# dyollb/segmantic

Hardware: AMD Instinct MI355X
Metric: 3D UNet train voxels/s on 128^3 bf16 (higher is better)
Workload: dtype bf16

## Files before the change

include/segmi.h:

```cpp
#ifndef SEGMI_H_
#define SEGMI_H_

#include <stddef.h>
#include <stdint.h>

#ifdef __cplusplus
extern "C" {
#endif

#define SEGMI_VERSION 1

enum { SEGMI_F32 = 0, SEGMI_BF16 = 1, SEGMI_F16 = 2 };
enum { SEGMI_OK = 0, SEGMI_EINVAL = -1, SEGMI_EUNSUPPORTED = -2, SEGMI_ELAUNCH = -3,
       SEGMI_EDATA = -4  };

typedef struct segmi_act {
  void* data;
  int32_t n, d, h, w;
  int32_t c;
  int32_t ld;
} segmi_act;

int segmi_version(void);
const char* segmi_last_error(void);
// ... 64 lines not shown
                     const segmi_bn_bwd_sums* bn_bwd ,
                     const segmi_bn_fin* stats_fin , void* stream);
int segmi_dectop_ok(int dtype, const segmi_act* in, const segmi_act* out);
int segmi_dectop_fwd(int dtype, const segmi_act* in, const segmi_act* out, const void* up_frag,
                     const float* up_bias, const float* up_alpha,
                     int up_alpha_in_unit_range ,
                     const void* conv_packed, const float* conv_bias, void* stream);
typedef struct segmi_windows {
  int32_t count;
  int32_t row_stride;
  int64_t plane_stride;
  int64_t offset[32];
} segmi_windows;
int segmi_conv3d_pair_ok(int dtype, const segmi_act* in, const segmi_act* out_a,
                         const segmi_act* out_b);
int segmi_conv3d_split_act_ok(int dtype, const segmi_act* in, const segmi_act* out, int ksize,
                              int stride);
int segmi_conv3d_fwd_split_act(int dtype, const segmi_act* in, const segmi_act* out,
                               const void* packed, const float* bias, const float* prelu_alpha,
                               int act_channels, int ksize, int stride,
                               const float* bias_b , float* stats_partials ,
                               const segmi_bn_fin* stats_fin , void* stream);
int segmi_conv3d_fwd_pair(int dtype, const segmi_act* in, const segmi_act* out_a, const float* w_a,
                          const float* bias_a, const float* prelu_alpha_a, float* stats_partials_a,
                          const segmi_act* out_b, const float* w_b, const float* bias_b, int stride,
                          const segmi_bn_fin* stats_fin_a ,
                          const segmi_windows* windows ,
                          void* stream);

int segmi_convT3d_stats_rows(int dtype, const segmi_act* in, const segmi_act* out);
int segmi_convT3d_fwd(int dtype, const segmi_act* in, const segmi_act* out, const void* packed,
                      const float* w_src, const float* bias, const float* prelu_alpha,
                      const segmi_act* residual, float* stats_partials,
                      const segmi_bn_fin* stats_fin , void* stream);

int64_t segmi_conv3d_wgrad_workspace(int dtype, const segmi_act* x, const segmi_act* dy,
                                     int ksize, int stride, int cus);
int segmi_conv3d_wgrad(int dtype, const segmi_act* x, const segmi_act* dy, float* dw,
                       float* db, int ksize, int stride, void* workspace,
                       const segmi_in_affine* in_tf , int cus, void* stream);
int segmi_wgrad_cus(int cus);
int segmi_bias_grad(int dtype, const segmi_act* dy, float* db, void* workspace, void* stream);

int segmi_bn_stats_rows(const segmi_act* x);
int segmi_bn_stats(int dtype, const segmi_act* x, float* stats_partials, void* stream);
int segmi_bn_finalize(const float* stats_partials, int rows, int c, double count,
                      const float* gamma, const float* beta, float* running_mean,
                      float* running_var, float momentum, float eps, float* mean,
                      float* invstd, float* scale, float* shift, void* stream);
int segmi_bn_eval_affine(int c, const float* gamma, const float* beta,
                         const float* running_mean, const float* running_var, float eps,
                         float* scale, float* shift, void* stream);
int segmi_bn_act_fwd(int dtype, const segmi_act* x, const segmi_act* y, const float* scale,
                     const float* shift, const float* prelu_alpha, const segmi_act* residual,
                     float dropout_p, uint32_t dropout_seed, void* stream);
int segmi_bn_act_bwd_rows(const segmi_act* x);
int segmi_bn_act_bwd_reduce(int dtype, const segmi_act* dy, const segmi_act* x,
                            const float* mean, const float* invstd, const float* gamma,
                            const float* beta, const float* prelu_alpha, float* red_partials,
                            float dropout_p, uint32_t dropout_seed,
                            const segmi_bn_bwd_fin* fin , void* stream);
int segmi_bn_act_bwd_finalize(const float* red_partials, int rows, int c, double count,
                              const float* gamma, const float* invstd, float* dgamma,
                              float* dbeta, float* dalpha, float* coef, void* stream);
int segmi_bn_act_bwd_fused_ok(int dtype, const segmi_act* dy, const segmi_act* x, const segmi_act* dx);
int segmi_bn_act_bwd_fused_rows(const segmi_act* x);
int segmi_bn_act_bwd_fused_wgs(int dtype, const segmi_act* x, int max_wgs);
int segmi_bn_act_bwd_fused(int dtype, const segmi_act* dy, const segmi_act* x, const segmi_act* dx,
                           const float* mean, const float* invstd, const float* gamma, const float* beta,
                           const float* prelu_alpha, float* red_partials, const segmi_bn_bwd_fin* fin,
                           int max_wgs, void* stream);
unsigned segmi_fused_timeouts(int reset);
int segmi_fused_test_hook(unsigned poll_limit, int no_publish);
int segmi_bn_act_bwd_apply(int dtype, const segmi_act* dy, const segmi_act* x,
                           const segmi_act* dx, const float* mean, const float* invstd,
                           const float* gamma, const float* beta, const float* prelu_alpha,
                           const float* coef, float dropout_p, uint32_t dropout_seed, void* stream);
int segmi_bn_act_bwd_apply_conv_ok(int dtype, const segmi_act* dy, const segmi_act* x, const segmi_act* dx,
                                   const segmi_act* out);
int segmi_bn_act_bwd_apply_conv(int dtype, const segmi_act* dy, const segmi_act* x, const segmi_act* dx,
                                const float* mean, const float* invstd, const float* gamma, const float* beta,
                                const float* prelu_alpha, const float* coef, const segmi_act* out,
                                const void* packed, void* stream);

int segmi_add(int dtype, const segmi_act* a, const segmi_act* b, const segmi_act* out,
              void* stream);
int segmi_cast_copy(int src_dtype, const segmi_act* src, int dst_dtype, const segmi_act* dst,
                    void* stream);
int segmi_nchw_to_ndhwc(const float* src, int dst_dtype, const segmi_act* dst, void* stream);
int segmi_ndhwc_to_nchw(int src_dtype, const segmi_act* src, float* dst, void* stream);

int segmi_dice_chunks(const segmi_act* logits);
int segmi_softmax_dice_fwd(int dtype, const segmi_act* logits, const float* labels,
                           float* partials, float* coef, float* loss, float smooth_nr,
                           float smooth_dr, void* stream);
int segmi_softmax_dice_bwd(int dtype, const segmi_act* logits, const float* labels,
                           const float* coef, float grad_scale, const segmi_act* dlogits,
                           float* scratch, float* bias_grad, void* stream);

int segmi_adam_step(float* param, const float* grad, float* exp_avg, float* exp_avg_sq,
                    float* max_exp_avg_sq, int64_t n, double lr, double beta1, double beta2,
                    double eps, double weight_decay, int64_t step, float grad_scale,
                    void* stream);
int segmi_sgd_step(float* param, const float* grad, float* momentum_buf, int64_t n, double lr,
                   double momentum, double weight_decay, int first_step, float grad_scale,
                   void* stream);
int segmi_adabelief_step(float* param, const float* grad, float* exp_avg, float* exp_avg_var,
                         int64_t n, double lr, double beta1, double beta2, double eps,
                         double weight_decay, int weight_decouple, int64_t step,
                         float grad_scale, void* stream);

int segmi_softmax_dice_bwd_amp(int dtype, const segmi_act* logits, const float* labels,
                               const float* coef, const float* amp, const segmi_act* dlogits,
                               float* scratch, float* bias_grad, void* stream);
int segmi_amp_check_finite(const float* grad, int64_t n, float* amp, void* stream);
int segmi_amp_update_scale(float* amp, int32_t* growth_tracker, int64_t* step, double growth_factor,
                           double backoff_factor, int growth_interval, void* stream);
int segmi_adam_step_amp(float* param, const float* grad, float* exp_avg, float* exp_avg_sq,
                        float* max_exp_avg_sq, int64_t n, double lr, double beta1, double beta2,
                        double eps, double weight_decay, const float* amp, const int64_t* step,
                        float grad_scale, void* stream);
int segmi_sgd_step_amp(float* param, const float* grad, float* momentum_buf, int64_t n, double lr,
                       double momentum, double weight_decay, const float* amp, const int64_t* step,
                       float grad_scale, void* stream);
int segmi_adabelief_step_amp(float* param, const float* grad, float* exp_avg, float* exp_avg_var,
                             int64_t n, double lr, double beta1, double beta2, double eps,
                             double weight_decay, int weight_decouple, const float* amp,
                             const int64_t* step, float grad_scale, void* stream);

int segmi_sw_gather(int dtype_src, const segmi_act* image, int img_index,
                    const int32_t* starts_host, int nwin, int dst_dtype,
                    const segmi_act* windows, void* stream);
int segmi_sw_scatter_add(int dtype, const segmi_act* pred, const int32_t* starts_host,
                         int nwin, const float* importance, const segmi_act* acc, float* cnt,
                         void* stream);
int segmi_sw_finalize(const segmi_act* acc, const float* cnt, int write_logits, void* labels,
                      int label_bytes, void* stream);
int segmi_sw_blend(int dtype, const void* cache, int k, int ldp, const int32_t* starts_z, int nz,
                   const int32_t* starts_y, int ny, const int32_t* starts_x, int nx, int win_lo,
                   int win_hi, int rd, int rh, int rw, const float* importance, int d, int h, int w,
                   float* out_logits, int ldo, float* out_count, void* labels, int label_bytes,
                   int normalize, void* stream);
int segmi_argmax(int dtype, const segmi_act* logits, void* labels, int label_bytes,
                 void* stream);
int segmi_label_counts(const int32_t* pred, const int32_t* truth, int64_t n, int k,
                       int64_t* counts, void* stream);

int segmi_resample3d(int pixel, const void* src, int sx, int sy, int sz, void* dst, int dx,
                     int dy, int dz, const double* index_map_host, int interp,
                     double default_value, void* stream);
int64_t segmi_normalize_workspace(int c, int64_t nvox);
int segmi_normalize_intensity(float* x, int c, int64_t nvox, void* workspace, void* stream);
int segmi_crop_patches(const segmi_act* image, const float* label, const int32_t* starts_host,
                       const uint8_t* flips_host, int count, int dst_dtype,
                       const segmi_act* out_image, float* out_label, void* stream);
int segmi_warp_crop_patches(const segmi_act* image, const float* label, const int32_t* starts_host,
                            const uint8_t* flips_host, int count, const double* index_map_host,
                            int dst_dtype, const segmi_act* out_image, float* out_label,
                            void* stream);
int64_t segmi_intensity_workspace(int count);
int segmi_intensity_augment(float* patches, int count, int rd, int rh, int rw, int c,
                            const uint8_t* contrast_on_host, const float* gamma_host,
                            const uint8_t* hist_on_host, const float* ctrl_host, int nctrl,
                            const uint8_t* bias_on_host, const float* coef_host, void* workspace,
                            void* stream);
int64_t segmi_kspace_workspace(int count, int rd, int rh, int rw);
// ... 70 lines not shown
```

segmantic_amd/_lib.py:

```python
from __future__ import annotations

import ctypes as C
import os
from pathlib import Path

import torch

SEGMI_F32 = 0
SEGMI_BF16 = 1
SEGMI_F16 = 2

_LIB_PATH = Path(__file__).resolve().parent / "csrc" / "libsegmi.so"


class Act(C.Structure):

    _fields_ = [("data", C.c_void_p), ("n", C.c_int32), ("d", C.c_int32), ("h", C.c_int32),
                ("w", C.c_int32), ("c", C.c_int32), ("ld", C.c_int32)]


class WpackDesc(C.Structure):

    _fields_ = [("w_src", C.c_void_p), ("scale", C.c_void_p), ("packed", C.c_void_p),
                ("kind", C.c_int32), ("cin_k", C.c_int32), ("cout_k", C.c_int32),
# ... 4 lines not shown
class InAffine(C.Structure):

    _fields_ = [("scale", C.c_void_p), ("shift", C.c_void_p), ("prelu_alpha", C.c_void_p)]


class Windows(C.Structure):

    _fields_ = [("count", C.c_int32), ("row_stride", C.c_int32), ("plane_stride", C.c_int64),
                ("offset", C.c_int64 * 32)]


class BnFin(C.Structure):

    _fields_ = [("count", C.c_double), ("gamma", C.c_void_p), ("beta", C.c_void_p),
                ("running_mean", C.c_void_p), ("running_var", C.c_void_p), ("momentum", C.c_float),
                ("eps", C.c_float), ("mean", C.c_void_p), ("invstd", C.c_void_p), ("scale", C.c_void_p),
                ("shift", C.c_void_p)]


class BnBwdFin(C.Structure):

    _fields_ = [("count", C.c_double), ("dgamma", C.c_void_p), ("dbeta", C.c_void_p), ("dalpha", C.c_void_p),
                ("coef", C.c_void_p)]


class BnBwdSums(C.Structure):

    _fields_ = [("x", C.POINTER(Act)), ("mean", C.c_void_p), ("invstd", C.c_void_p), ("gamma", C.c_void_p),
                ("beta", C.c_void_p), ("prelu_alpha", C.c_void_p), ("partials", C.c_void_p),
                ("fin", C.POINTER(BnBwdFin))]


_P = C.c_void_p
_AP = C.POINTER(Act)
_i = C.c_int
_i64 = C.c_int64
_f = C.c_float
_d = C.c_double

SIGNATURES = {
    "segmi_version": (_i, []),
    "segmi_last_error": (C.c_char_p, []),
    "segmi_stream_create_cumask": (_i, [_i, C.POINTER(C.c_void_p)]),
    "segmi_stream_destroy": (_i, [_P]),
    "segmi_wpack_bytes": (_i64, [_i, _i, _i, _i, _i]),
    "segmi_wpack": (_i, [_i, _i, _P, _P, _i, _i, _i, _P, _P]),
    "segmi_wpack_batch": (_i, [_i, C.POINTER(WpackDesc), _i, _P, _i, _P]),
    "segmi_conv3d_stats_rows": (_i, [_i, _AP, _AP, _i, _i]),
    "segmi_conv3d_in_affine_ok": (_i, [_i, _AP, _AP, _i, _i]),
    "segmi_conv3d_fwd_kernel_name": (C.c_char_p, [_i, _AP, _AP, _i, _i]),
    "segmi_conv3d_split_act_ok": (_i, [_i, _AP, _AP, _i, _i]),
    "segmi_conv3d_fwd_split_act": (_i, [_i, _AP, _AP, _P, _P, _P, _i, _i, _i, _P, _P, C.POINTER(BnFin), _P]),
    "segmi_conv3d_fwd": (_i, [_i, _AP, _AP, _P, _P, _i, _P, _P, _AP, _P, _i, _i, C.POINTER(InAffine),
                              C.POINTER(BnBwdSums), C.POINTER(BnFin), _P]),
    "segmi_conv3d_bn_bwd_sums_ok": (_i, [_i, _AP, _AP, _i, _i]),
    "segmi_dectop_ok": (_i, [_i, _AP, _AP]),
    "segmi_dectop_fwd": (_i, [_i, _AP, _AP, _P, _P, _P, _i, _P, _P, _P]),
    "segmi_conv3d_pair_ok": (_i, [_i, _AP, _AP, _AP]),
    "segmi_conv3d_fwd_pair": (_i, [_i, _AP, _AP, _P, _P, _P, _P, _AP, _P, _P, _i, C.POINTER(BnFin),
                                   C.POINTER(Windows), _P]),
    "segmi_convT3d_stats_rows": (_i, [_i, _AP, _AP]),
    "segmi_convT3d_fwd": (_i, [_i, _AP, _AP, _P, _P, _P, _P, _AP, _P, C.POINTER(BnFin), _P]),
    "segmi_conv3d_wgrad_workspace": (_i64, [_i, _AP, _AP, _i, _i, _i]),
    "segmi_conv3d_wgrad": (_i, [_i, _AP, _AP, _P, _P, _i, _i, _P, C.POINTER(InAffine), _i, _P]),
    "segmi_bias_grad": (_i, [_i, _AP, _P, _P, _P]),
    "segmi_bn_stats_rows": (_i, [_AP]),
    "segmi_bn_stats": (_i, [_i, _AP, _P, _P]),
    "segmi_bn_finalize": (_i, [_P, _i, _i, _d, _P, _P, _P, _P, _f, _f, _P, _P, _P, _P, _P]),
    "segmi_bn_eval_affine": (_i, [_i, _P, _P, _P, _P, _f, _P, _P, _P]),
    "segmi_bn_act_fwd": (_i, [_i, _AP, _AP, _P, _P, _P, _AP, _f, C.c_uint32, _P]),
    "segmi_bn_act_bwd_rows": (_i, [_AP]),
    "segmi_bn_act_bwd_reduce": (_i, [_i, _AP, _AP, _P, _P, _P, _P, _P, _P, _f, C.c_uint32,
                                     C.POINTER(BnBwdFin), _P]),
    "segmi_bn_act_bwd_finalize": (_i, [_P, _i, _i, _d, _P, _P, _P, _P, _P, _P, _P]),
    "segmi_bn_act_bwd_fused_ok": (_i, [_i, _AP, _AP, _AP]),
    "segmi_bn_act_bwd_fused_rows": (_i, [_AP]),
    "segmi_bn_act_bwd_fused": (_i, [_i, _AP, _AP, _AP, _P, _P, _P, _P, _P, _P, C.POINTER(BnBwdFin), _i, _P]),
    "segmi_bn_act_bwd_fused_wgs": (_i, [_i, _AP, _i]),
    "segmi_fused_timeouts": (C.c_uint, [_i]),
    "segmi_fused_test_hook": (_i, [C.c_uint, _i]),
    "segmi_bn_act_bwd_apply": (_i, [_i, _AP, _AP, _AP, _P, _P, _P, _P, _P, _P, _f, C.c_uint32, _P]),
    "segmi_bn_act_bwd_apply_conv_ok": (_i, [_i, _AP, _AP, _AP, _AP]),
    "segmi_bn_act_bwd_apply_conv": (_i, [_i, _AP, _AP, _AP, _P, _P, _P, _P, _P, _P, _AP, _P, _P]),
    "segmi_wgrad_cus": (_i, [_i]),
    "segmi_add": (_i, [_i, _AP, _AP, _AP, _P]),
    "segmi_cast_copy": (_i, [_i, _AP, _i, _AP, _P]),
    "segmi_nchw_to_ndhwc": (_i, [_P, _i, _AP, _P]),
    "segmi_ndhwc_to_nchw": (_i, [_i, _AP, _P, _P]),
    "segmi_dice_chunks": (_i, [_AP]),
    "segmi_softmax_dice_fwd": (_i, [_i, _AP, _P, _P, _P, _P, _f, _f, _P]),
    "segmi_softmax_dice_bwd": (_i, [_i, _AP, _P, _P, _f, _AP, _P, _P, _P]),
    "segmi_adam_step": (_i, [_P, _P, _P, _P, _P, _i64, _d, _d, _d, _d, _d, _i64, _f, _P]),
    "segmi_sgd_step": (_i, [_P, _P, _P, _i64, _d, _d, _d, _i, _f, _P]),
    "segmi_adabelief_step": (_i, [_P, _P, _P, _P, _i64, _d, _d, _d, _d, _d, _i, _i64, _f, _P]),
    "segmi_softmax_dice_bwd_amp": (_i, [_i, _AP, _P, _P, _P, _AP, _P, _P, _P]),
    "segmi_amp_check_finite": (_i, [_P, _i64, _P, _P]),
    "segmi_amp_update_scale": (_i, [_P, _P, _P, _d, _d, _i, _P]),
    "segmi_adam_step_amp": (_i, [_P, _P, _P, _P, _P, _i64, _d, _d, _d, _d, _d, _P, _P, _f, _P]),
    "segmi_sgd_step_amp": (_i, [_P, _P, _P, _i64, _d, _d, _d, _P, _P, _f, _P]),
    "segmi_adabelief_step_amp": (_i, [_P, _P, _P, _P, _i64, _d, _d, _d, _d, _d, _i, _P, _P, _f, _P]),
    "segmi_sw_gather": (_i, [_i, _AP, _i, _P, _i, _i, _AP, _P]),
    "segmi_sw_scatter_add": (_i, [_i, _AP, _P, _i, _P, _AP, _P, _P]),
    "segmi_sw_finalize": (_i, [_AP, _P, _i, _P, _i, _P]),
    "segmi_sw_blend": (_i, [_i, _P, _i, _i, _P, _i, _P, _i, _P, _i, _i, _i, _i, _i, _i, _P, _i, _i, _i,
                            _P, _i, _P, _P, _i, _i, _P]),
    "segmi_argmax": (_i, [_i, _AP, _P, _i, _P]),
    "segmi_label_counts": (_i, [_P, _P, _i64, _i, _P, _P]),
    "segmi_resample3d": (_i, [_i, _P, _i, _i, _i, _P, _i, _i, _i, _P, _i, _d, _P]),
    "segmi_normalize_workspace": (_i64, [_i, _i64]),
    "segmi_normalize_intensity": (_i, [_P, _i, _i64, _P, _P]),
    "segmi_crop_patches": (_i, [_AP, _P, _P, _P, _i, _i, _AP, _P, _P]),
    "segmi_warp_crop_patches": (_i, [_AP, _P, _P, _P, _i, _P, _i, _AP, _P, _P]),
    "segmi_intensity_workspace": (_i64, [_i]),
    "segmi_intensity_augment": (_i, [_P, _i, _i, _i, _i, _i, _P, _P, _P, _P, _i, _P, _P, _P, _P]),
    "segmi_ensemble_mean": (_i, [_P, _P, _i, _i64, _P, _P]),
    "segmi_ensemble_vote": (_i, [_P, _i, _i64, _P, _P]),
    "segmi_ensemble_select": (_i, [_P, _i, _P, _P, _i, _i64, _P, _P]),
    "segmi_kspace_workspace": (_i64, [_i, _i, _i, _i]),
    "segmi_kspace_augment": (_i, [_P, _i, _i, _i, _i, _i, _P, _P, _P, _P, _P, _P, _P, _P]),
    "segmi_label_boxes": (_i, [_P, _P, _i, _i, _i, _i, _i, _P, _P, _P]),
    "segmi_edt_workspace_bytes": (_i64, [_i, _i, _i]),
    "segmi_edt_sq": (_i, [_P, _i, _i, _i, _i, _i, _i, _i, _P, _P, _P, _P, C.c_size_t, _P]),
    "segmi_edt_sample": (_i, [_P, _P, _i, _i, _i, _i, _i, _i, _i, _P, _P, _P, _P, _P, C.c_size_t, _P]),
    "segmi_select_workspace_bytes": (_i64, [_i]),
    "segmi_select_f32": (_i, [_P, _P, _P, _i, _P, _P, C.c_size_t, _P]),
    "segmi_confusion_counts": (_i, [_P, _P, _i, _i64, _i, _P, _P]),
    "segmi_nyul_workspace_bytes": (_i64, [_i, _i]),
    "segmi_nyul_landmarks": (_i, [_P, _i, _i64, _i, _P, _i, _P, _P, _P, C.c_size_t, _P]),
    "segmi_nyul_apply": (_i, [_P, _i, _i64, _i, _P, _P, _P, _i, _P]),
    "segmi_label_centroids": (_i, [_P, _i, _i, _i, _i, _i, _P, _P, _P]),
    "segmi_vert_heatmap": (_i, [_P, _i, _P, _P, _i, _i, _i, _i, _P, _P]),
    "segmi_channel_argmax": (_i, [_P, _i, _i, _i, _i, _P, _P, _P]),
    "segmi_positive_bbox": (_i, [_P, _i, _i, _i, _i, _i, _i, _P, _P]),
    "segmi_otsu_workspace_bytes": (_i64, [_i]),
    "segmi_otsu": (_i, [_P, _i64, _i, _P, _P, _P, C.c_size_t, _P]),
    "segmi_n4_shrink": (_i, [_P, _i, _i, _i, _i, _i, _i, _P, _P, _i, _i, _P, _P, _P, _P]),
    "segmi_n4_workspace_bytes": (_i64, [_i, _i, _i, _i, _i, _i]),
    "segmi_n4_fit": (_i, [_P, _i, _i, _i, _P, _i, _i, _i, _d, _d, _d, _P, _P, _P, _P, _P, C.c_size_t, _P]),
    "segmi_n4_sharpen": (_i, [_P, _i, _i, _i, _i, _d, _d, _P, _P, _P, C.c_size_t, _P]),
    "segmi_n4_bspline_fit": (_i, [_P, _i, _i, _i, _i, _P, _P, C.c_size_t, _P]),
    "segmi_n4_refine": (_i, [_P, _i, _i, _i, _P, _P]),
    "segmi_n4_evaluate": (_i, [_P, _i, _i, _i, _P, _P, _i, _i, _i, _P]),
    "segmi_ct_scale": (_i, [_P, _i, _i, _i, _P, _P]),
}


def _load():
    path = Path(os.environ.get("SEGMI_LIB", str(_LIB_PATH)))
    if not path.exists():
        raise ImportError(
            f"segmantic_amd: native library {path} not found. Build it with "
            f"`python -c 'import __graft_entry__ as g; g.build()'` or `make -C segmantic_amd/csrc`. "
            f"There is no CPU fallback.")
    try:
        lib = C.CDLL(str(path))
    except OSError as e:
        raise ImportError(f"segmantic_amd: cannot load {path}: {e}") from e
    missing = []
    for name, (res, args) in SIGNATURES.items():
        try:
            fn = getattr(lib, name)
        except AttributeError:
            missing.append(name)
            continue
        fn.restype = res
        fn.argtypes = args
# ... 16 lines not shown
```

segmantic_amd/csrc/conv.hip:

```cpp
#include "conv_fwd_impl.h"
#include "conv_ring_impl.h"
#include "conv_ks_impl.h"
#include "convt_ps_impl.h"
#include "conv_bnbwd_impl.h"

namespace segmi {

int conv_s2_bnbwd_bf16(const ConvBnBwdParams& p, hipStream_t st);
int conv_s2_bnbwd_f16(const ConvBnBwdParams& p, hipStream_t st);

int conv_mfma_f32(const ConvParams& p, int ksize, int stride, hipStream_t st);
int conv_mfma_bf16(const ConvParams& p, int ksize, int stride, hipStream_t st);
int conv_mfma_f16(const ConvParams& p, int ksize, int stride, hipStream_t st);
int convt_mfma_f32(const ConvTParams& p, hipStream_t st);
int convt_mfma_bf16(const ConvTParams& p, hipStream_t st);
int convt_mfma_f16(const ConvTParams& p, hipStream_t st);
static inline int conv_mfma_dt(int dtype, const ConvParams& p, int ksize, int stride, hipStream_t st) {
  if (dtype == SEGMI_F32) return conv_mfma_f32(p, ksize, stride, st);
  return dtype == SEGMI_F16 ? conv_mfma_f16(p, ksize, stride, st) : conv_mfma_bf16(p, ksize, stride, st);
}
static inline int convt_mfma_dt(int dtype, const ConvTParams& p, hipStream_t st) {
  if (dtype == SEGMI_F32) return convt_mfma_f32(p, st);
  return dtype == SEGMI_F16 ? convt_mfma_f16(p, st) : convt_mfma_bf16(p, st);
}
int bn_stats_launch(int dtype, const segmi_act* x, float* partials, hipStream_t st, const BiasFin* bias_fin = nullptr);
int bn_stats_rows_for(const segmi_act* x);
int stats_reserve_rows();
static inline int bn_finalize_with(const float* partials, int rows, int c, const segmi_bn_fin* f, hipStream_t st) {
  return segmi_bn_finalize(partials, rows, c, f->count, f->gamma, f->beta, f->running_mean, f->running_var,
                           f->momentum, f->eps, f->mean, f->invstd, f->scale, f->shift, st);
}
bool conv_small_ok(int cin, int cout, int ksize);
int conv_small_fwd(int dtype, const segmi_act* in, const segmi_act* out, const float* w,
                   const float* bias, const float* alpha, const segmi_act* res, float* stats,
                   int stride, hipStream_t st, const segmi_act* out2 = nullptr,
                   const float* w2 = nullptr, const float* bias2 = nullptr,
                   const segmi_bn_fin* fin = nullptr, const segmi_windows* win = nullptr);
int conv_small_fwd_rows(const segmi_act* out);

struct DirectParams {
  const void* in;
  void* out;
  const float* w;
  const float* bias;
  const float* alpha;
  const void* res;
  int N, Di, Hi, Wi, Do, Ho, Wo, Cin, Cout, ldi, ldo, ldr;
  int ks, stride, kind;
};

template <typename T>
__global__ void conv_direct_kernel(DirectParams p) {
  const int64_t total = (int64_t)p.N * p.Do * p.Ho * p.Wo * p.Cout;
  const int pad = (p.ks - 1) / 2, nt = p.ks * p.ks * p.ks;
  const T* in = (const T*)p.in;
  for (int64_t e = blockIdx.x * (int64_t)blockDim.x + threadIdx.x; e < total;
       e += (int64_t)gridDim.x * blockDim.x) {
    const int co = e % p.Cout;
    int64_t v = e / p.Cout;
    const int ox = v % p.Wo; v /= p.Wo;
    const int oy = v % p.Ho; v /= p.Ho;
    const int oz = v % p.Do;
    const int n = v / p.Do;
    float acc = 0.f;
    for (int kd = 0; kd < p.ks; ++kd) {
      const int z = oz * p.stride - pad + kd;
      if ((unsigned)z >= (unsigned)p.Di) continue;
      for (int kh = 0; kh < p.ks; ++kh) {
        const int y = oy * p.stride - pad + kh;
        if ((unsigned)y >= (unsigned)p.Hi) continue;
        for (int kw = 0; kw < p.ks; ++kw) {
          const int x = ox * p.stride - pad + kw;
          if ((unsigned)x >= (unsigned)p.Wi) continue;
          const int tap = (kd * p.ks + kh) * p.ks + kw;
          const T* ip = in + ((((int64_t)n * p.Di + z) * p.Hi + y) * p.Wi + x) * p.ldi;
          if (p.kind == 0) {
            const float* wp = p.w + ((int64_t)co * p.Cin) * nt + tap;
            for (int ci = 0; ci < p.Cin; ++ci) acc = fmaf(Elem<T>::ld(ip + ci), wp[(int64_t)ci * nt], acc);
          } else {
            const float* wp = p.w + (int64_t)co * nt + (nt - 1 - tap);
            for (int ci = 0; ci < p.Cin; ++ci)
              acc = fmaf(Elem<T>::ld(ip + ci), wp[(int64_t)ci * p.Cout * nt], acc);
          }
        }
      }
    }
    if (p.bias) acc += p.bias[co];
// ... 128 lines not shown
                  "conv3d_fwd_split_act: act_channels must be a multiple of 16 within the output channels");
  SEGMI_CHECK_ARG(in->n == out->n && out->d == out_extent(in->d, ksize, stride) &&
                      out->h == out_extent(in->h, ksize, stride) && out->w == out_extent(in->w, ksize, stride),
                  "conv3d_fwd_split_act: output extent does not match the input");
  const int es = dtype_size(dtype);
  SEGMI_CHECK_ARG(in->ld % (16 / es) == 0 && out->ld % 4 == 0 && ((uintptr_t)in->data % 16) == 0 &&
                      ((uintptr_t)out->data % (4 * es)) == 0,
                  "conv3d_fwd_split_act: MFMA path needs 16-byte aligned input rows");
  ConvParams p{};
  p.in = in->data; p.out = out->data; p.wfrag = packed; p.bias = bias; p.alpha = prelu_alpha;
  p.N = in->n; p.Di = in->d; p.Hi = in->h; p.Wi = in->w;
  p.Do = out->d; p.Ho = out->h; p.Wo = out->w;
  p.Cin = in->c; p.Cout = out->c; p.ldi = in->ld; p.ldo = out->ld;
  p.nchunks = in->c / pick_ck(dtype, in->c);
  p.ntiles_total = out->c / 16;
  p.act_tiles = act_channels / 16;
  p.bias2 = bias_b;
  if (stats_partials) {
    p.stats = stats_partials;
    p.stats_tiles = act_channels / 16;
    if (stats_fin) { p.fin_on = 1; p.bfin = bn_fin_from(stats_fin, act_channels); }
  } else {
    SEGMI_CHECK_ARG(!stats_fin, "conv3d_fwd_split_act: stats_fin needs stats_partials");
  }
  hipStream_t st = (hipStream_t)stream;
  return conv_mfma_dt(dtype, p, ksize, stride, st);
}

const char* segmi_conv3d_fwd_kernel_name(int dtype, const segmi_act* in, const segmi_act* out,
                                         int ksize, int stride) {
  static thread_local char buf[96];
  if (!act_ok(in) || !act_ok(out)) return "invalid";
  const char* dt = dtype == SEGMI_BF16 ? "bf16" : dtype == SEGMI_F16 ? "f16" : "f32";
  if (mfma_ok(in->c, out->c)) {
    const int ck = pick_ck(dtype, in->c);
    if (conv_ring_ok(dtype, in->c, ksize, stride, out)) {
      if (conv_ring3_shape_ok(in->c, out->c, in->data, out->data, in->d, in->h, in->w, in->ld, out->d, out->h, out->w, out->ld,
                              out->ld, out->ld))
        snprintf(buf, sizeof buf, "conv_ring3_kernel<%s, CK=16> (LDS-DMA ring)", dt);
      else
        snprintf(buf, sizeof buf, "conv_ring2_kernel<%s, CK=%d, NT=%d>", dt, ck,
                 ck == 32 && (out->c / 16) % 2 == 0 ? 2 : 1);
    }
    else if (conv_ks_ok(dtype, in->c, ksize, stride))
      snprintf(buf, sizeof buf, "conv_fwd_ks_kernel<%s, k%d s%d>", dt, ksize, stride);
    else
      snprintf(buf, sizeof buf, "conv_fwd_mfma_kernel<%s, CK=%d, k%d s%d>", dt, ck, ksize, stride);
    return buf;
  }
  if (small_fwd_eligible(dtype, in, out, ksize)) snprintf(buf, sizeof buf, "conv_small_fwd_kernel<%s>", dt);
  else snprintf(buf, sizeof buf, "conv_direct_kernel<%s>", dt);
  return buf;
}

int segmi_conv3d_in_affine_ok(int dtype, const segmi_act* in, const segmi_act* out, int ksize,
                              int stride) {
  if (!act_ok(in) || !act_ok(out) || !dtype_h16(dtype) || !mfma_ok(in->c, out->c)) return 0;
  return ksize == 3 && stride == 1 && conv_ring_ok(dtype, in->c, ksize, stride, out) ? 1 : 0;
}

int segmi_conv3d_bn_bwd_sums_ok(int dtype, const segmi_act* in, const segmi_act* out, int ksize,
                                int stride) {
  if (!act_ok(in) || !act_ok(out) || !dtype_h16(dtype)) return 0;
  return ((in->c == 16 && out->c == 16) || (in->c == 32 && out->c == 32)) && ksize == 3 && stride == 1 &&
                 conv_ring_ok(dtype, in->c, ksize, stride, out) ? 1 : 0;
}

int segmi_bn_act_bwd_apply_conv_ok(int dtype, const segmi_act* dy, const segmi_act* x, const segmi_act* dx,
                                   const segmi_act* out) {
  if (!dtype_h16(dtype) || !act_ok(dy) || !act_ok(x) || !act_ok(dx) || !act_ok(out)) return 0;
  const segmi_act* a3[3] = {dy, x, dx};
  for (const segmi_act* a : a3) {
    if (a->n != dy->n || a->d != dy->d || a->h != dy->h || a->w != dy->w || a->c != 16) return 0;
    if (a->ld % 8 != 0 || ((uintptr_t)a->data % 16) != 0) return 0;
  }
  if (out->n != dy->n || out->d != out_extent(dy->d, 3, 2) || out->h != out_extent(dy->h, 3, 2) ||
      out->w != out_extent(dy->w, 3, 2))
    return 0;
  if (!(out->c == 16 || out->c == 32 || out->c == 64) || out->ld % 4 != 0 || ((uintptr_t)out->data % 8) != 0)
    return 0;
  const int64_t vox = (int64_t)dy->d * dy->h * dy->w;
  if (vox * dy->ld * 2 >= (1ll << 31) || vox * x->ld * 2 >= (1ll << 31) || vox * dx->ld * 2 >= (1ll << 31)) return 0;
  return out->w >= 16 ? 1 : 0;
}

int segmi_bn_act_bwd_apply_conv(int dtype, const segmi_act* dy, const segmi_act* x, const segmi_act* dx,
                                const float* mean, const float* invstd, const float* gamma, const float* beta,
                                const float* prelu_alpha, const float* coef, const segmi_act* out,
                                const void* packed, void* stream) {
  SEGMI_CHECK_ARG(segmi_bn_act_bwd_apply_conv_ok(dtype, dy, x, dx, out) && mean && invstd && coef && packed,
                  "bn_act_bwd_apply_conv: not eligible (ask segmi_bn_act_bwd_apply_conv_ok) or bad arguments");
  SEGMI_CHECK_ARG(dx->data != dy->data && dx->data != x->data,
                  "bn_act_bwd_apply_conv: dx must not alias dy or x (halo voxels are re-read by neighbouring tiles)");
  ConvBnBwdParams p{};
  p.dy = dy->data; p.x = x->data; p.dx = dx->data; p.out = out->data; p.wfrag = packed;
  p.mean = mean; p.invstd = invstd; p.gamma = gamma; p.beta = beta; p.alpha = prelu_alpha; p.coef = coef;
  p.N = dy->n; p.Di = dy->d; p.Hi = dy->h; p.Wi = dy->w; p.Do = out->d; p.Ho = out->h; p.Wo = out->w;
  p.Cout = out->c; p.ldy = dy->ld; p.ldx = x->ld; p.lddx = dx->ld; p.ldo = out->ld;
  p.ntiles_total = out->c / 16;
  return dtype == SEGMI_F16 ? conv_s2_bnbwd_f16(p, (hipStream_t)stream) : conv_s2_bnbwd_bf16(p, (hipStream_t)stream);
}

int segmi_conv3d_fwd(int dtype, const segmi_act* in, const segmi_act* out, const void* packed,
                     const float* w_src, int w_kind, const float* bias,
                     const float* prelu_alpha, const segmi_act* residual,
                     float* stats_partials, int ksize, int stride, const segmi_in_affine* in_tf,
                     const segmi_bn_bwd_sums* bn_bwd, const segmi_bn_fin* stats_fin, void* stream) {
  SEGMI_CHECK_ARG(!stats_fin || (stats_partials && bn_fin_ok(stats_fin)),
                  "conv3d: stats_fin needs stats_partials and its output pointers");
  if (bn_bwd && bn_bwd->fin)
    SEGMI_CHECK_ARG(bn_bwd->fin->count > 0 && bn_bwd->fin->coef, "conv3d: bn_bwd->fin needs count and coef");
  if (bn_bwd)
    SEGMI_CHECK_ARG(bn_bwd->x && act_ok(bn_bwd->x) && bn_bwd->mean && bn_bwd->invstd && bn_bwd->partials &&
                        segmi_conv3d_bn_bwd_sums_ok(dtype, in, out, ksize, stride) && !prelu_alpha &&
                        !stats_partials && bn_bwd->x->n == out->n && bn_bwd->x->d == out->d &&
                        bn_bwd->x->h == out->h && bn_bwd->x->w == out->w && bn_bwd->x->c == out->c &&
                        bn_bwd->x->ld % 4 == 0 && ((uintptr_t)bn_bwd->x->data % 8) == 0,
                    "conv3d: this launch cannot take BatchNorm-backward sums (ask segmi_conv3d_bn_bwd_sums_ok)");
  if (in_tf)
    SEGMI_CHECK_ARG(in_tf->scale && in_tf->shift && segmi_conv3d_in_affine_ok(dtype, in, out, ksize, stride),
                    "conv3d: this layer cannot take an input transform (ask segmi_conv3d_in_affine_ok)");
  SEGMI_CHECK_ARG(dtype_ok(dtype), "conv3d: bad dtype %d", dtype);
  SEGMI_CHECK_ARG(act_ok(in) && act_ok(out), "conv3d: bad activation view");
  SEGMI_CHECK_ARG((ksize == 1 || ksize == 3) && (stride == 1 || stride == 2),
                  "conv3d: unsupported ksize/stride %d/%d", ksize, stride);
  SEGMI_CHECK_ARG(!(ksize == 1 && stride != 1), "conv3d: k1 is stride 1 only");
  SEGMI_CHECK_ARG(in->n == out->n && out->d == out_extent(in->d, ksize, stride) &&
                      out->h == out_extent(in->h, ksize, stride) &&
                      out->w == out_extent(in->w, ksize, stride),
                  "conv3d: output extent [%d,%d,%d,%d] does not match input [%d,%d,%d,%d] k%d s%d",
                  out->n, out->d, out->h, out->w, in->n, in->d, in->h, in->w, ksize, stride);
  if (residual)
    SEGMI_CHECK_ARG(act_ok(residual) && residual->n == out->n && residual->d == out->d &&
                        residual->h == out->h && residual->w == out->w && residual->c == out->c,
                    "conv3d: residual shape mismatch");
  hipStream_t st = (hipStream_t)stream;
  const int es = dtype_size(dtype);
  if (mfma_ok(in->c, out->c)) {
    SEGMI_CHECK_ARG(packed, "conv3d: MFMA path needs a fragment-packed weight (segmi_wpack)");
    SEGMI_CHECK_ARG(in->ld % (16 / es) == 0 && out->ld % 4 == 0 &&
                        ((uintptr_t)in->data % 16) == 0 && ((uintptr_t)out->data % (4 * es)) == 0,
                    "conv3d: MFMA path needs 16-byte aligned input rows");
    if (residual)
      SEGMI_CHECK_ARG(residual->ld % 4 == 0 && ((uintptr_t)residual->data % (4 * es)) == 0,
                      "conv3d: residual rows must be 4-element aligned");
    ConvParams p{};
    p.in = in->data; p.out = out->data; p.wfrag = packed; p.bias = bias; p.alpha = prelu_alpha;
    p.res = residual ? residual->data : nullptr; p.stats = stats_partials;
    p.N = in->n; p.Di = in->d; p.Hi = in->h; p.Wi = in->w;
    p.Do = out->d; p.Ho = out->h; p.Wo = out->w;
    p.Cin = in->c; p.Cout = out->c; p.ldi = in->ld; p.ldo = out->ld;
    p.ldr = residual ? residual->ld : 0;
    p.nchunks = in->c / pick_ck(dtype, in->c);
    p.ntiles_total = out->c / 16;
    if (in_tf) { p.in_scale = in_tf->scale; p.in_shift = in_tf->shift; p.in_alpha = in_tf->prelu_alpha; }
    if (bn_bwd) {
      p.bx = bn_bwd->x->data; p.ldbx = bn_bwd->x->ld; p.bmean = bn_bwd->mean; p.binvstd = bn_bwd->invstd;
      p.bgamma = bn_bwd->gamma; p.bbeta = bn_bwd->beta; p.balpha = bn_bwd->prelu_alpha;
      p.bpart = bn_bwd->partials;
      SEGMI_CHECK_ARG((int64_t)p.Ho * p.Wo * p.ldbx < (1ll << 31), "conv3d: plane too large for 32-bit offsets");
      if (bn_bwd->fin) {
        p.fin_on = 1;
        p.bbfin = BnBwdFin{out->c, bn_bwd->fin->count, bn_bwd->fin->dgamma, bn_bwd->fin->dbeta,
                           bn_bwd->fin->dalpha, bn_bwd->fin->coef};
      }
    }
// ... 107 lines not shown
```

segmantic_amd/csrc/conv_mfma_h16.h:

```cpp
#pragma once
#include "conv_fwd_impl.h"
#include "conv_ring2_impl.h"
#include "conv_ring3_impl.h"
#include "conv_ks_impl.h"
#include "convt_ps_impl.h"
#include "conv_bnbwd_impl.h"
namespace segmi {
template <typename T>
static int conv_mfma_h16(const ConvParams& p, int ksize, int stride, hipStream_t st) {
  constexpr int dt = DtypeOf<T>::value;
  if (conv_ring_zsplit(dt, p.Cin, ksize, stride, p.N, p.Do, p.Ho, p.Wo) > 0)
    return conv_ring3_ok(p) ? launch_conv_ring3<T>(p, st) : launch_conv_ring2<T>(p, st);
  if (conv_ks_ok(dt, p.Cin, ksize, stride)) return launch_conv_ks_t<T, 32>(p, st);
  return launch_conv_mfma_t<T>(p, ksize, stride, st);
}
template <typename T>
static int conv_s2_bnbwd_h16(const ConvBnBwdParams& p, hipStream_t st) {
  switch (p.Cout / 16) {
    case 1: return launch_conv_s2_bnbwd<T, 1>(p, st);
    case 2: return launch_conv_s2_bnbwd<T, 2>(p, st);
    case 4: return launch_conv_s2_bnbwd<T, 4>(p, st);
  }
  SEGMI_UNSUPPORTED("bn_act_bwd_apply_conv: %d output channels", p.Cout);
}
template <typename T>
static int convt_mfma_h16(const ConvTParams& p, hipStream_t st) {
  if (convt_ps_ok(DtypeOf<T>::value, p.Cin, p.Cout, p.Wi)) return launch_convt_ps_t<T>(p, st);
  return launch_convt_mfma_t<T>(p, st);
}
}
```

segmantic_amd/ops.py:

```python
from __future__ import annotations

import ctypes as C
from typing import Optional, Sequence

import numpy as np
import torch

from . import _lib
from ._lib import SEGMI_BF16, SEGMI_F16, SEGMI_F32, Act, BnBwdFin, BnBwdSums, BnFin, InAffine, Windows, check, lib

_DT = {torch.float32: SEGMI_F32, torch.bfloat16: SEGMI_BF16, torch.float16: SEGMI_F16}


def dtype_code(t: torch.Tensor) -> int:
    try:
        return _DT[t.dtype]
    except KeyError:
        raise TypeError(f"unsupported activation dtype {t.dtype} (float32 / bfloat16 / float16 only)")


def _stream() -> int:
    return torch.cuda.current_stream().cuda_stream


# ... 300 lines not shown
    check(lib.segmi_bn_eval_affine(running_mean.numel(), _ptr(gamma), _ptr(beta),
                                   _ptr(running_mean), _ptr(running_var), eps, _ptr(scale),
                                   _ptr(shift), _stream()), "bn_eval_affine")


def bn_act_fwd(x, y, scale, shift, prelu_alpha=None, residual=None, dropout=(0.0, 0)) -> None:
    ax, ay = act(x), act(y)
    ar = act(residual) if residual is not None else None
    check(lib.segmi_bn_act_fwd(dtype_code(x), C.byref(ax), C.byref(ay), _ptr(scale),
                               _ptr(shift), _ptr(prelu_alpha), _ref(ar), float(dropout[0]),
                               int(dropout[1]) & 0xFFFFFFFF, _stream()),
          "bn_act_fwd")


def bn_act_bwd_rows(x) -> int:
    ax = act(x)
    return int(lib.segmi_bn_act_bwd_rows(C.byref(ax)))


def bn_act_bwd_reduce(dy, x, mean, invstd, gamma, beta, prelu_alpha, partials,
                      dropout=(0.0, 0), fin=None) -> None:
    ady, ax = act(dy), act(x)
    bf = _bn_bwd_fin(fin)
    check(lib.segmi_bn_act_bwd_reduce(dtype_code(x), C.byref(ady), C.byref(ax), _ptr(mean),
                                      _ptr(invstd), _ptr(gamma), _ptr(beta), _ptr(prelu_alpha),
                                      _ptr(partials), float(dropout[0]), int(dropout[1]) & 0xFFFFFFFF,
                                      C.byref(bf) if bf is not None else None, _stream()), "bn_act_bwd_reduce")


def bn_act_bwd_fused_ok(dy, x, dx) -> bool:
    ady, ax, adx = act(dy), act(x), act(dx)
    return bool(lib.segmi_bn_act_bwd_fused_ok(dtype_code(x), C.byref(ady), C.byref(ax), C.byref(adx)))


def bn_act_bwd_fused_rows(x) -> int:
    a = act(x)
    return int(lib.segmi_bn_act_bwd_fused_rows(C.byref(a)))


def bn_act_bwd_fused(dy, x, dx, mean, invstd, gamma, beta, prelu_alpha, partials, fin, max_wgs: int = 0) -> None:
    ady, ax, adx = act(dy), act(x), act(dx)
    bf = _bn_bwd_fin(fin)
    check(lib.segmi_bn_act_bwd_fused(dtype_code(x), C.byref(ady), C.byref(ax), C.byref(adx), _ptr(mean),
                                     _ptr(invstd), _ptr(gamma), _ptr(beta), _ptr(prelu_alpha), _ptr(partials),
                                     C.byref(bf), int(max_wgs), _stream()), "bn_act_bwd_fused")


def bn_act_bwd_fused_wgs(x, max_wgs: int = 0) -> int:
    a = act(x)
    return int(lib.segmi_bn_act_bwd_fused_wgs(dtype_code(x), C.byref(a), int(max_wgs)))


def fused_timeouts(reset: bool = False) -> int:
    return int(lib.segmi_fused_timeouts(1 if reset else 0))


def check_fused_timeouts(where: str = "") -> None:
    n = fused_timeouts(reset=True)
    if n:
        raise RuntimeError(
            f"{n} workgroup(s) of segmi_bn_act_bwd_fused gave up waiting for their launch's last workgroup"
            f"{' (' + where + ')' if where else ''}: the launch was never fully resident (GPU shared with another "
            "process, or CUs masked).  The gradients of that step are NaN and the weights are poisoned: restart "
            "from the last checkpoint with SEGMI_FUSE_BN_BWD_SMALL=0 (three launches, no grid-wide wait).")


def fused_test_hook(poll_limit: int = 0, no_publish: bool = False) -> None:
    check(lib.segmi_fused_test_hook(int(poll_limit), 1 if no_publish else 0), "fused_test_hook")


def bn_act_bwd_apply_conv_ok(dy, x, dx, out) -> bool:
    ady, ax, adx, ao = act(dy), act(x), act(dx), act(out)
    return bool(lib.segmi_bn_act_bwd_apply_conv_ok(dtype_code(x), C.byref(ady), C.byref(ax), C.byref(adx),
                                                   C.byref(ao)))


def bn_act_bwd_apply_conv(dy, x, dx, mean, invstd, gamma, beta, prelu_alpha, coef, out, packed) -> None:
    ady, ax, adx, ao = act(dy), act(x), act(dx), act(out)
    check(lib.segmi_bn_act_bwd_apply_conv(dtype_code(x), C.byref(ady), C.byref(ax), C.byref(adx), _ptr(mean),
                                          _ptr(invstd), _ptr(gamma), _ptr(beta), _ptr(prelu_alpha), _ptr(coef),
                                          C.byref(ao), _ptr(packed), _stream()), "bn_act_bwd_apply_conv")


def bn_act_bwd_finalize(partials, rows, c, count, gamma, invstd, dgamma, dbeta, dalpha,
                        coef) -> None:
    check(lib.segmi_bn_act_bwd_finalize(_ptr(partials), rows, c, float(count), _ptr(gamma),
                                        _ptr(invstd), _ptr(dgamma), _ptr(dbeta), _ptr(dalpha),
                                        _ptr(coef), _stream()), "bn_act_bwd_finalize")


def bn_act_bwd_apply(dy, x, dx, mean, invstd, gamma, beta, prelu_alpha, coef,
                     dropout=(0.0, 0)) -> None:
    ady, ax, adx = act(dy), act(x), act(dx)
    check(lib.segmi_bn_act_bwd_apply(dtype_code(x), C.byref(ady), C.byref(ax), C.byref(adx),
                                     _ptr(mean), _ptr(invstd), _ptr(gamma), _ptr(beta),
                                     _ptr(prelu_alpha), _ptr(coef), float(dropout[0]),
                                     int(dropout[1]) & 0xFFFFFFFF, _stream()),
          "bn_act_bwd_apply")


def add(a, b, out) -> None:
    aa, ao = act(a), act(out)
    ab = act(b) if b is not None else None
    check(lib.segmi_add(dtype_code(a), C.byref(aa), _ref(ab), C.byref(ao), _stream()), "add")


def cast_copy(src, dst) -> None:
    a, b = act(src), act(dst)
    check(lib.segmi_cast_copy(dtype_code(src), C.byref(a), dtype_code(dst), C.byref(b),
                              _stream()), "cast_copy")


def nchw_to_ndhwc(src: torch.Tensor, dst: torch.Tensor) -> None:
    if src.dtype != torch.float32 or not src.is_contiguous():
        raise ValueError("nchw_to_ndhwc expects a contiguous float32 NCDHW tensor")
    b = act(dst)
    check(lib.segmi_nchw_to_ndhwc(_ptr(src), dtype_code(dst), C.byref(b), _stream()),
          "nchw_to_ndhwc")


def ndhwc_to_nchw(src: torch.Tensor, dst: torch.Tensor) -> None:
    a = act(src)
    if dst.dtype != torch.float32 or not dst.is_contiguous():
        raise ValueError("ndhwc_to_nchw writes a contiguous float32 NCDHW tensor")
    check(lib.segmi_ndhwc_to_nchw(dtype_code(src), C.byref(a), _ptr(dst), _stream()),
          "ndhwc_to_nchw")


def dice_chunks(logits) -> int:
    a = act(logits)
    return int(lib.segmi_dice_chunks(C.byref(a)))


def softmax_dice_fwd(logits, labels, partials, coef, loss, smooth_nr=1e-5, smooth_dr=1e-5):
    a = act(logits)
    check(lib.segmi_softmax_dice_fwd(dtype_code(logits), C.byref(a), _ptr(labels),
                                     _ptr(partials), _ptr(coef), _ptr(loss), smooth_nr,
                                     smooth_dr, _stream()), "softmax_dice_fwd")


def softmax_dice_bwd(logits, labels, coef, grad_scale, dlogits, scratch=None, bias_grad=None) -> None:
    a, b = act(logits), act(dlogits)
    check(lib.segmi_softmax_dice_bwd(dtype_code(logits), C.byref(a), _ptr(labels), _ptr(coef),
                                     float(grad_scale), C.byref(b), _ptr(scratch), _ptr(bias_grad),
                                     _stream()),
          "softmax_dice_bwd")


def adam_step(param, grad, exp_avg, exp_avg_sq, max_exp_avg_sq, lr, beta1, beta2, eps,
              weight_decay, step, grad_scale=1.0) -> None:
    check(lib.segmi_adam_step(_ptr(param), _ptr(grad), _ptr(exp_avg), _ptr(exp_avg_sq),
                              _ptr(max_exp_avg_sq), param.numel(), lr, beta1, beta2, eps,
                              weight_decay, step, grad_scale, _stream()), "adam_step")


def sgd_step(param, grad, buf, lr, momentum, weight_decay, first_step, grad_scale=1.0) -> None:
    check(lib.segmi_sgd_step(_ptr(param), _ptr(grad), _ptr(buf), param.numel(), lr, momentum,
                             weight_decay, int(first_step), grad_scale, _stream()), "sgd_step")


def adabelief_step(param, grad, exp_avg, exp_avg_var, lr, beta1, beta2, eps, weight_decay,
                   weight_decouple, step, grad_scale=1.0) -> None:
    check(lib.segmi_adabelief_step(_ptr(param), _ptr(grad), _ptr(exp_avg), _ptr(exp_avg_var),
                                   param.numel(), lr, beta1, beta2, eps, weight_decay,
                                   int(weight_decouple), step, grad_scale, _stream()),
          "adabelief_step")
# ... 579 lines not shown
```

Measured before the change: 3.605 billion.

## Add z-marching LDS ring kernel for fused BN-backward plus stride-2 conv

Adds a ring-buffer variant of the fused BN/activation backward apply plus stride-2 3x3x3 convolution. Each workgroup marches along depth over a column tile and keeps three input planes in LDS, so overlapping halo planes between consecutive output slices are loaded and BN-applied once instead of recomputed. Weights sit in LDS, and the depth axis is split to fill the CUs. The kernel is dispatched for Cout 32/64 when the split heuristic allows, at the cost of more LDS, a lower occupancy bound and extra barriers per step.

```diff
diff --git a/include/segmi.h b/include/segmi.h
--- a/include/segmi.h
+++ b/include/segmi.h
@@ -170,6 +170,8 @@
                                 const float* mean, const float* invstd, const float* gamma, const float* beta,
                                 const float* prelu_alpha, const float* coef, const segmi_act* out,
                                 const void* packed, void* stream);
+const char* segmi_bn_act_bwd_apply_conv_kernel_name(int dtype, const segmi_act* dy, const segmi_act* x,
+                                                    const segmi_act* dx, const segmi_act* out);
 
 int segmi_add(int dtype, const segmi_act* a, const segmi_act* b, const segmi_act* out,
               void* stream);
diff --git a/segmantic_amd/_lib.py b/segmantic_amd/_lib.py
--- a/segmantic_amd/_lib.py
+++ b/segmantic_amd/_lib.py
@@ -110,6 +110,7 @@
     "segmi_bn_act_bwd_apply": (_i, [_i, _AP, _AP, _AP, _P, _P, _P, _P, _P, _P, _f, C.c_uint32, _P]),
     "segmi_bn_act_bwd_apply_conv_ok": (_i, [_i, _AP, _AP, _AP, _AP]),
     "segmi_bn_act_bwd_apply_conv": (_i, [_i, _AP, _AP, _AP, _P, _P, _P, _P, _P, _P, _AP, _P, _P]),
+    "segmi_bn_act_bwd_apply_conv_kernel_name": (C.c_char_p, [_i, _AP, _AP, _AP, _AP]),
     "segmi_wgrad_cus": (_i, [_i]),
     "segmi_add": (_i, [_i, _AP, _AP, _AP, _P]),
     "segmi_cast_copy": (_i, [_i, _AP, _i, _AP, _P]),
diff --git a/segmantic_amd/csrc/conv.hip b/segmantic_amd/csrc/conv.hip
--- a/segmantic_amd/csrc/conv.hip
+++ b/segmantic_amd/csrc/conv.hip
@@ -3,6 +3,7 @@
 #include "conv_ks_impl.h"
 #include "convt_ps_impl.h"
 #include "conv_bnbwd_impl.h"
+#include "conv_bnbwd_ring_impl.h"
 
 namespace segmi {
 
@@ -297,6 +298,13 @@
   const int64_t vox = (int64_t)dy->d * dy->h * dy->w;
   if (vox * dy->ld * 2 >= (1ll << 31) || vox * x->ld * 2 >= (1ll << 31) || vox * dx->ld * 2 >= (1ll << 31)) return 0;
   return out->w >= 16 ? 1 : 0;
+}
+
+const char* segmi_bn_act_bwd_apply_conv_kernel_name(int dtype, const segmi_act* dy, const segmi_act* x,
+                                                    const segmi_act* dx, const segmi_act* out) {
+  if (!segmi_bn_act_bwd_apply_conv_ok(dtype, dy, x, dx, out)) return "not eligible";
+  return conv_s2_bnbwd_ring_zsplit(dy->n, out->d, out->h, out->w, out->c) > 0 ? "conv_s2_bnbwd_ring_kernel"
+                                                                              : "conv_s2_bnbwd_kernel";
 }
 
 int segmi_bn_act_bwd_apply_conv(int dtype, const segmi_act* dy, const segmi_act* x, const segmi_act* dx,
diff --git a/segmantic_amd/csrc/conv_bnbwd_ring_impl.h b/segmantic_amd/csrc/conv_bnbwd_ring_impl.h
--- /dev/null
+++ b/segmantic_amd/csrc/conv_bnbwd_ring_impl.h
@@ -0,0 +1,219 @@
+#pragma once
+#include "conv_bnbwd_impl.h"
+
+namespace segmi {
+
+struct BnBwdRingGeom {
+  static constexpr int TH = 4, TW = 16;
+  static constexpr int HH = 2 * TH + 1, HW = 2 * TW + 1;
+  static constexpr int ROWB = 32;
+  static constexpr int PLANE_VOX = HH * HW;
+  static constexpr int PLANE_B = PLANE_VOX * ROWB;
+  static constexpr int STEP_VOX = 2 * PLANE_VOX;
+  static constexpr int KB = (STEP_VOX + 127) / 128;
+  static constexpr int NSTEP = 14;
+  static constexpr int RING_B = 3 * PLANE_B;
+  template <int NT> static constexpr int w_bytes() { return NSTEP * NT * 1024; }
+  template <int NT> static constexpr int lds_bytes() { return w_bytes<NT>() + RING_B; }
+};
+
+static inline int conv_s2_bnbwd_ring_zsplit(int N, int Do, int Ho, int Wo, int Cout) {
+  using G = BnBwdRingGeom;
+  if (!(Cout == 32 || Cout == 64) || Wo < G::TW || Do < 4) return 0;
+  const int per_cu = Cout == 32 ? 2 : 1;
+  const int64_t columns = (int64_t)N * cdiv(Ho, G::TH) * cdiv(Wo, G::TW);
+  int tz = (int)((256 * per_cu + columns - 1) / columns);
+  if (tz < 1) tz = 1;
+  if (tz > Do / 4) tz = Do / 4;
+  const int64_t wgs = columns * tz;
+  if (wgs < 256 * per_cu || wgs >= (1ll << 31)) return 0;
+  return tz;
+}
+
+template <typename T, int NT>
+__global__ __launch_bounds__(256, NT <= 2 ? 2 : 1) void conv_s2_bnbwd_ring_kernel(ConvBnBwdParams p) {
+  using G = BnBwdRingGeom;
+  constexpr int KB = G::KB;
+  constexpr int W_B = G::w_bytes<NT>();
+  constexpr int RING = W_B;
+  constexpr unsigned kOob = 0x80000000u;
+  extern __shared__ __attribute__((aligned(16))) char smem[];
+  const int tid = threadIdx.x, lane = tid & 63;
+  const int wave = __builtin_amdgcn_readfirstlane(tid >> 6);
+  const int g = lane >> 4, r = lane & 15;
+
+  int t = blockIdx.x;
+  const int seg = t % p.tz; t /= p.tz;
+  const int txi = t % p.tx; t /= p.tx;
+  const int tyi = t % p.ty;
+  const int n = t / p.ty;
+  const int oy0 = tyi * G::TH, ox0 = txi * G::TW;
+  const int seg_len = (p.Do + p.tz - 1) / p.tz;
+  const int oza = seg * seg_len;
+  const int ozb = oza + seg_len < p.Do ? oza + seg_len : p.Do;
+  if (oza >= ozb) return;
+
+  {
+    const char* wsrc = (const char*)p.wfrag;
+#pragma unroll
+    for (int i = 0; i < W_B / 4096; ++i)
+      *reinterpret_cast<frag_t*>(smem + 4096 * i + 16 * tid) = *reinterpret_cast<const frag_t*>(wsrc + 4096 * i + 16 * tid);
+  }
+
+  const int half = wave & 1;
+  const int c8 = half * 8;
+  f32x2 m2[4], i2[4], g2[4], b2[4], c02[4], c12[4], gi2[4];
+#pragma unroll
+  for (int q = 0; q < 4; ++q)
+#pragma unroll
+    for (int h = 0; h < 2; ++h) {
+      const int ch = c8 + 2 * q + h;
+      m2[q][h] = p.mean[ch];
+      i2[q][h] = p.invstd[ch];
+      g2[q][h] = p.gamma ? p.gamma[ch] : 1.f;
+      b2[q][h] = p.beta ? p.beta[ch] : 0.f;
+      c02[q][h] = p.coef[ch];
+      c12[q][h] = p.coef[16 + ch];
+    }
+#pragma unroll
+  for (int q = 0; q < 4; ++q) {
+    gi2[q] = g2[q] * i2[q];
+    asm volatile("" : "+v"(gi2[q]), "+v"(b2[q]));
+  }
+  const bool has_alpha = p.alpha != nullptr;
+  const float alpha = has_alpha ? *p.alpha : 1.f;
+
+  const int64_t svox = (int64_t)p.Di * p.Hi * p.Wi;
+  const __amdgpu_buffer_rsrc_t rs_dy = __builtin_amdgcn_make_buffer_rsrc(
+      (void*)((const char*)p.dy + (n * svox * p.ldy + c8) * 2), 0, (int)(svox * p.ldy * 2 - c8 * 2), 0x00020000);
+  const __amdgpu_buffer_rsrc_t rs_x = __builtin_amdgcn_make_buffer_rsrc(
+      (void*)((const char*)p.x + (n * svox * p.ldx + c8) * 2), 0, (int)(svox * p.ldx * 2 - c8 * 2), 0x00020000);
+  const __amdgpu_buffer_rsrc_t rs_dx = __builtin_amdgcn_make_buffer_rsrc(
+      (void*)((char*)p.dx + (n * svox * p.lddx + c8) * 2), 0, (int)(svox * p.lddx * 2 - c8 * 2), 0x00020000);
+  const int pvox = p.Hi * p.Wi;
+  const unsigned pb_dy = (unsigned)pvox * p.ldy * 2, pb_x = (unsigned)pvox * p.ldx * 2, pb_dx = (unsigned)pvox * p.lddx * 2;
+  int ofy[KB], ofx[KB], ofd[KB];
+  int pl[KB];
+  unsigned lo[KB];
+  const int vbase = (wave >> 1) * 64 + lane;
+#pragma unroll
+  for (int k = 0; k < KB; ++k) {
+    const int v = vbase + 128 * k;
+    const int pk = v / G::PLANE_VOX, rem = v % G::PLANE_VOX;
+    const int hy = rem / G::HW, hx = rem % G::HW;
+    const int y = 2 * oy0 - 1 + hy, x = 2 * ox0 - 1 + hx;
+    const bool ok = (v < G::STEP_VOX) & ((unsigned)y < (unsigned)p.Hi) & ((unsigned)x < (unsigned)p.Wi);
+    const int vox = y * p.Wi + x;
+    ofy[k] = ok ? vox * p.ldy * 2 : -1;
+    ofx[k] = vox * p.ldx * 2;
+    ofd[k] = vox * p.lddx * 2;
+    pl[k] = (pk & 1) | (((hy >= 1) & (hx >= 1)) ? 2 : 0);
+    lo[k] = (unsigned)(rem * G::ROWB + half * 16);
+  }
+  const int zlo = 2 * oza - 1;
+
+  frag_t dzr[KB], xr[KB];
+  int code[KB];
+  auto issue = [&](int zf) __attribute__((always_inline)) {
+#pragma unroll
+    for (int k = 0; k < KB; ++k) {
+      const int z = zf + (pl[k] & 1);
+      const bool inside = (ofy[k] >= 0) & (z >= zlo) & ((unsigned)z < (unsigned)p.Di);
+      code[k] = inside ? ((pl[k] & 1) << 1) | (int)(((pl[k] >> 1) & 1) & (z > zlo)) : -1;
+      dzr[k] = __builtin_amdgcn_raw_buffer_load_b128(rs_dy, inside ? (unsigned)z * pb_dy + (unsigned)ofy[k] : kOob, 0, 0);
+      xr[k] = __builtin_amdgcn_raw_buffer_load_b128(rs_x, inside ? (unsigned)z * pb_x + (unsigned)ofx[k] : kOob, 0, 0);
+    }
+  };
+  auto commit = [&](int zf, auto ha) __attribute__((always_inline)) {
+    constexpr bool HA = decltype(ha)::value;
+    const unsigned s0 = RING + (unsigned)(((zf + 3) % 3) * G::PLANE_B), s1 = RING + (unsigned)(((zf + 4) % 3) * G::PLANE_B);
+#pragma unroll
+    for (int k = 0; k < KB; ++k) {
+      frag_t val;
+#pragma unroll
+      for (int q = 0; q < 4; ++q) {
+        const f32x2 a{H16<T>::lo(xr[k][q]), H16<T>::hi(xr[k][q])};
+        const f32x2 d{H16<T>::lo(dzr[k][q]), H16<T>::hi(dzr[k][q])};
+        const f32x2 o2 = bn_bwd_apply_elem2g<HA>(a, d, m2[q], i2[q], g2[q], b2[q], c02[q], c12[q], gi2[q], alpha);
+        val[q] = code[k] >= 0 ? H16<T>::pack2(o2[0], o2[1]) : 0u;
+      }
+      const int z = zf + (pl[k] & 1);
+      const bool own = (code[k] >= 0) & ((code[k] & 1) != 0);
+      __builtin_amdgcn_raw_buffer_store_b128(val, rs_dx, own ? (unsigned)z * pb_dx + (unsigned)ofd[k] : kOob, 0, 0);
+      if (k < KB - 1 || vbase + 128 * k < G::STEP_VOX)
+        *reinterpret_cast<frag_t*>(smem + ((pl[k] & 1) ? s1 : s0) + lo[k]) = val;
+    }
+  };
+
+  auto tap_off = [&](int tp) __attribute__((always_inline)) { return ((2 * wave + (tp / 3) % 3) * G::HW + 2 * r + tp % 3) * G::ROWB + (g & 1) * 16; };
+  T* outp = (T*)p.out;
+  const int oy = oy0 + wave, ox = ox0 + r;
+  const bool row_ok = oy < p.Ho && ox < p.Wo;
+  const char* wl = smem + lane * 16;
+
+  auto march = [&](auto ha) __attribute__((always_inline)) {
+    issue(zlo - 1);
+    commit(zlo - 1, ha);
+    __syncthreads();
+    issue(2 * oza);
+    commit(2 * oza, ha);
+    __syncthreads();
+    for (int oz = oza; oz < ozb; ++oz) {
+      const bool more = oz + 1 < ozb;
+      if (more) issue(2 * oz + 2);
+      const unsigned sb0 = RING + (unsigned)(((2 * oz + 2) % 3) * G::PLANE_B);
+      const unsigned sb1 = RING + (unsigned)(((2 * oz) % 3) * G::PLANE_B);
+      const unsigned sb2 = RING + (unsigned)(((2 * oz + 1) % 3) * G::PLANE_B);
+      f32x4 acc[NT];
+#pragma unroll
+      for (int j = 0; j < NT; ++j) acc[j] = f32x4{0.f, 0.f, 0.f, 0.f};
+#pragma unroll
+      for (int s = 0; s < G::NSTEP; ++s) {
+        const int t0 = 2 * s, t1 = 2 * s + 1 < 27 ? 2 * s + 1 : 0;
+        const unsigned b0 = t0 / 9 == 0 ? sb0 : t0 / 9 == 1 ? sb1 : sb2;
+        const unsigned b1 = t1 / 9 == 0 ? sb0 : t1 / 9 == 1 ? sb1 : sb2;
+        const unsigned addr = (g >> 1) ? b1 + (unsigned)tap_off(t1 % 9) : b0 + (unsigned)tap_off(t0 % 9);
+        const frag_t a = *reinterpret_cast<const frag_t*>(smem + addr);
+#pragma unroll
+        for (int j = 0; j < NT; ++j) {
+          const frag_t wf = *reinterpret_cast<const frag_t*>(wl + (s * NT + j) * 1024);
+          acc[j] = mma16<T>(wf, a, acc[j]);
+        }
+      }
+      if (row_ok) {
+        const int64_t v = (((int64_t)n * p.Do + oz) * p.Ho + oy) * p.Wo + ox;
+#pragma unroll
+        for (int j = 0; j < NT; ++j) store4<T>(outp + v * p.ldo + j * 16 + 4 * g, acc[j]);
+      }
+      if (more) {
+        __syncthreads();
+        commit(2 * oz + 2, ha);
+        __syncthreads();
+      }
+    }
+  };
+  if (has_alpha) march(std::true_type{});
+  else march(std::false_type{});
+}
+
+template <typename T, int NT>
+static int launch_conv_s2_bnbwd_ring(ConvBnBwdParams p, int tz, hipStream_t st) {
+  using G = BnBwdRingGeom;
+  p.tz = tz;
+  p.ty = cdiv(p.Ho, G::TH);
+  p.tx = cdiv(p.Wo, G::TW);
+  const int64_t nb = (int64_t)p.N * p.ty * p.tx * p.tz;
+  constexpr int lds = G::lds_bytes<NT>();
+  static_assert(G::w_bytes<NT>() % 4096 == 0, "the weight copy moves 4 KiB per pass");
+  auto kern = conv_s2_bnbwd_ring_kernel<T, NT>;
+  static bool attr_done = false;
+  if (!attr_done) {
+    (void)hipFuncSetAttribute(reinterpret_cast<const void*>(kern), hipFuncAttributeMaxDynamicSharedMemorySize, lds);
+    attr_done = true;
+  }
+  hipLaunchKernelGGL(kern, dim3((unsigned)nb), 256, lds, st, p);
+  SEGMI_LAUNCH_CHECK("bn_act_bwd_apply_conv(ring)");
+  return SEGMI_OK;
+}
+
+}
diff --git a/segmantic_amd/csrc/conv_mfma_h16.h b/segmantic_amd/csrc/conv_mfma_h16.h
--- a/segmantic_amd/csrc/conv_mfma_h16.h
+++ b/segmantic_amd/csrc/conv_mfma_h16.h
@@ -5,6 +5,7 @@
 #include "conv_ks_impl.h"
 #include "convt_ps_impl.h"
 #include "conv_bnbwd_impl.h"
+#include "conv_bnbwd_ring_impl.h"
 namespace segmi {
 template <typename T>
 static int conv_mfma_h16(const ConvParams& p, int ksize, int stride, hipStream_t st) {
@@ -16,6 +17,10 @@
 }
 template <typename T>
 static int conv_s2_bnbwd_h16(const ConvBnBwdParams& p, hipStream_t st) {
+  if (const int tz = conv_s2_bnbwd_ring_zsplit(p.N, p.Do, p.Ho, p.Wo, p.Cout)) {
+    if (p.Cout == 32) return launch_conv_s2_bnbwd_ring<T, 2>(p, tz, st);
+    return launch_conv_s2_bnbwd_ring<T, 4>(p, tz, st);
+  }
   switch (p.Cout / 16) {
     case 1: return launch_conv_s2_bnbwd<T, 1>(p, st);
     case 2: return launch_conv_s2_bnbwd<T, 2>(p, st);
diff --git a/segmantic_amd/ops.py b/segmantic_amd/ops.py
--- a/segmantic_amd/ops.py
+++ b/segmantic_amd/ops.py
@@ -406,6 +406,12 @@
                                           C.byref(ao), _ptr(packed), _stream()), "bn_act_bwd_apply_conv")
 
 
+def bn_act_bwd_apply_conv_kernel_name(dy, x, dx, out) -> str:
+    ady, ax, adx, ao = act(dy), act(x), act(dx), act(out)
+    return lib.segmi_bn_act_bwd_apply_conv_kernel_name(dtype_code(x), C.byref(ady), C.byref(ax), C.byref(adx),
+                                                       C.byref(ao)).decode()
+
+
 def bn_act_bwd_finalize(partials, rows, c, count, gamma, invstd, dgamma, dbeta, dalpha,
                         coef) -> None:
     check(lib.segmi_bn_act_bwd_finalize(_ptr(partials), rows, c, float(count), _ptr(gamma),
```

Result: faster. 3.662 billion, median of 6 (+1.6%).
